# nikizadehgfdl/ocean_model_grid_generator

Measured on AMD Instinct MI355X. Metric: supergrid cells/sec (coords+metrics), 1/8° tripolar at 1/2/4/8 MI355X, higher is better.
Workload: dtype f64

## Files before the change

include/ogg_hip.h:

```cpp
#ifndef OGG_HIP_H
#define OGG_HIP_H

#ifdef __cplusplus
extern "C" {
#endif

#define OGG_OK 0
#define OGG_EORDER 1
#define OGG_ESHAPE 2
#define OGG_EHIP 3
#define OGG_ENOMEM 4
#define OGG_EARG 5

#define OGG_DP_ARC_LITERAL 0
#define OGG_DP_ARC_CHORD 1

#define OGG_SYM_DEFAULT 0
#define OGG_SYM_MIRROR 1
#define OGG_SYM_NONE 2

const char* ogg_last_error(void);
const char* ogg_version(void);
long ogg_abi_sizeof(int which);
int ogg_device_count(int* count);
// ... 177 lines not shown
    long workspace_bytes;
    int symmetry;
} ogg_dpole_band;
long ogg_dpole_band_workspace_bytes(int order, long Ni, long n_pt_rows);
int ogg_symmetry_coverage(int which, int order, long n, double lon0, double lon_dp, int symmetry, int* cell_writes, int* col_writes,
                          long* evaluated);
int ogg_supergrid_pass_dev(int n_latlon, const ogg_latlon_band* latlon, long ni1, double lon0, double lenlon, double Re, int metrics,
                           const ogg_bipolar_band* cap, const ogg_dpole_band* south_cap, void** events5, double* alg_bytes4,
                           void* stream);
int ogg_supergrid_pass_plan_dev(int n_latlon, const ogg_latlon_band* latlon, long ni1, double lon0, double lenlon, double Re, int metrics,
                                const ogg_bipolar_band* cap, const ogg_dpole_band* south_cap, void** plan_out);
int ogg_supergrid_pass_run_dev(void* plan, void** events5, double* alg_bytes4, void* stream);
int ogg_supergrid_pass_plan_destroy(void* plan);
long ogg_supergrid_pass_plan_slots(const void* plan);
long ogg_supergrid_pass_plan_carried_runs(const void* plan);
int ogg_supergrid_pass_plan_flags_dev(const void* plan, int* flags, void* stream);

int ogg_fill_dev(long n, double value, double* out, void* stream);
int ogg_bswap64_dev(long n, const void* src, void* dst, void* stream);
int ogg_libm_check_dev(int which, long n, const double* x, const double* y, unsigned long long* n_diff, void* stream);
#define OGG_MATH_DIV_PI180 0
#define OGG_MATH_RCP_C3 1
#define OGG_MATH_RSQRT_C3 2
#define OGG_MATH_ATAN_SERIES14 3
#define OGG_MATH_ATAN_SERIES17 4
#define OGG_MATH_ATAN_CAP 5
#define OGG_MATH_ATAN2_ANGLE 6
#define OGG_MATH_WAVE_PREV 7
#define OGG_MATH_WAVE_NEXT 8
#define OGG_MATH_WAVE_PREV_TAIL 9
// ... 372 lines not shown
```

ocean_model_grid_generator_amd/_lib.py:

```python
import ctypes
import os

import numpy as np

_HERE = os.path.dirname(os.path.abspath(__file__))
LIB_PATH = os.environ.get("OGG_LIB_PATH") or os.path.join(_HERE, "csrc", "libogg_hip.so")

OGG_OK, OGG_EORDER, OGG_ESHAPE, OGG_EHIP, OGG_ENOMEM, OGG_EARG = 0, 1, 2, 3, 4, 5
DP_ARC_LITERAL, DP_ARC_CHORD = 0, 1
SYM_DEFAULT, SYM_MIRROR, SYM_NONE = 0, 1, 2

MATH = {"div_pi180": 0, "rcp_c3": 1, "rsqrt_c3": 2, "atan_series14": 3, "atan_series17": 4, "atan_cap": 5, "atan2_angle": 6,
        "wave_prev": 7, "wave_next": 8, "wave_prev_tail": 9, "wave_next_tail": 10, "xcd_contiguous": 11, "lib_atan": 12, "atan_lib": 13, "wave_next_int": 14,
        "sin_tiny": 32, "asin_tiny": 33, "cos_cap": 34, "hom_arc": 35, "hom_tan": 36, "lib_sin": 37, "lib_asin": 38, "lib_cos": 39}

c_long, c_int, c_double, c_void_p, c_longlong = ctypes.c_long, ctypes.c_int, ctypes.c_double, ctypes.c_void_p, ctypes.c_longlong
_dp = ctypes.POINTER(ctypes.c_double)
_llp = ctypes.POINTER(ctypes.c_longlong)

class LatlonBand(ctypes.Structure):
    _fields_ = [("axis_kind", c_int), ("a0", c_double), ("len", c_double), ("denom", c_double), ("y0", c_longlong),
                ("lat1d", c_void_p), ("k0", c_long), ("n_pt_rows", c_long), ("n_cell_rows", c_long), ("x", c_void_p),
                ("y", c_void_p), ("dx", c_void_p), ("dy", c_void_p), ("area", c_void_p), ("angle", c_void_p)]

# ... 364 lines not shown
    "ogg_event_create": [ctypes.POINTER(c_void_p)],
    "ogg_event_destroy": [c_void_p],
    "ogg_event_record": [c_void_p, c_void_p],
    "ogg_event_elapsed_ms": [c_void_p, c_void_p, ctypes.POINTER(ctypes.c_float)],
    "ogg_stream_synchronize": [c_void_p],
}
STRING_GETTERS = ("ogg_last_error", "ogg_version")
LONG_GETTERS = {"ogg_abi_sizeof": [c_int],
                "ogg_bipolar_quad_workspace_bytes": [c_int, c_long, c_long],
                "ogg_displaced_pole_quad_workspace_bytes": [c_int, c_long, c_long],
                "ogg_displaced_pole_grid_workspace_bytes": [c_long, c_long],
                "ogg_dpole_band_workspace_bytes": [c_int, c_long, c_long],
                "ogg_latlon_rows_workspace_bytes": [c_int, ctypes.POINTER(LatlonBand), c_long],
                "ogg_supergrid_pass_plan_slots": [c_void_p],
                "ogg_supergrid_pass_plan_carried_runs": [c_void_p],
                "ogg_grid_quality_result_bytes": [],
                "ogg_grid_quality_workspace_bytes": [c_long, c_long],
                "ogg_topog_record_bytes": [],
                "ogg_topog_plane_record_bytes": [],
                "ogg_topog_band_out_rows": [ctypes.POINTER(TopogBand)],
                "ogg_topog_workspace_bytes": [],
                "ogg_xgrid_struct_bytes": [c_int],
                "ogg_xgrid_band_first_row": [ctypes.POINTER(XgridBand)],
                "ogg_xgrid_band_out_rows": [ctypes.POINTER(XgridBand)],
                "ogg_xgrid_band_next_rows": [ctypes.POINTER(XgridBand)],
                "ogg_xgrid_workspace_bytes": [ctypes.POINTER(XgridBand), ctypes.POINTER(XgridAtm)],
                "ogg_mask_struct_bytes": [c_int],
                "ogg_mask_workspace_bytes": [ctypes.POINTER(MaskParams)],
                "ogg_remap_struct_bytes": [c_int],
                "ogg_remap_workspace_bytes": [ctypes.POINTER(RemapParams)],
# ... 91 lines not shown
```

ocean_model_grid_generator_amd/csrc/ogg_latlon_fused_dev.h:

```cpp
#pragma once
#include <cmath>
#include <cstdlib>

#include "../../include/ogg_hip.h"
#include "ogg_common.h"
#include "ogg_math.h"

namespace {
using namespace ogg;

constexpr int LF_TX = 256;
constexpr int LF_ROWS = 32;
constexpr int LF_MAX_BANDS = 4;

struct RowScalars {
    double lat, sl, cl, dy;
};

struct FusedParams {
    int n_bands;
    ogg_latlon_band band[LF_MAX_BANDS];
    long strip0[LF_MAX_BANDS + 1];
    long ni1;
    double lon0, lenlon, Ni;
    int rows_per_block;
    double Re, Re2;
    int metrics;
    const RowScalars* row_tab;
    long row0[LF_MAX_BANDS + 1];
};

OGG_DEV double axis_lat(const ogg_latlon_band& b, long k, double Ni) {
    if (b.axis_kind == 0) return b.a0 + ((double)k * b.len) / b.denom;
    if (b.axis_kind == 1) {
        const double R = Ni / (2 * kPi);
        return atan(sinh((double)(b.y0 + k) / R)) * k180Pi;
    }
    return b.lat1d[k];
}

OGG_DEV RowScalars latlon_row_scalars(const FusedParams& f, const ogg_latlon_band& b, long j) {
    const long n_cell_rows = f.metrics ? b.n_cell_rows : 0;
    RowScalars r = {0.0, 0.0, 0.0, 0.0};
    if (j < b.n_pt_rows || j - 1 < n_cell_rows) {
        r.lat = axis_lat(b, b.k0 + j, f.Ni);
        const double lv = (0.5 * (r.lat + r.lat)) * kPi180;
        sincos(lv, &r.sl, &r.cl);
        if (j < n_cell_rows) {
            const double dyj = (axis_lat(b, b.k0 + j + 1, f.Ni) - r.lat) * kPi180;
            r.dy = f.Re * sqrt(dyj * dyj + 0.0);
        }
    }
    return r;
}

OGG_DEV void latlon_row_table_body(const FusedParams& f, long b, long n_wg) {
    const long n_rows = f.row0[f.n_bands];
    RowScalars* tab = const_cast<RowScalars*>(f.row_tab);
    for (long k = b * LF_TX + threadIdx.x; k < n_rows; k += n_wg * LF_TX) {
        int bi = 0;
        while (bi + 1 < f.n_bands && k >= f.row0[bi + 1]) ++bi;
        tab[k] = latlon_row_scalars(f, f.band[bi], k - f.row0[bi]);
    }
}
inline long latlon_row_table_blocks(const FusedParams& f) { return f.n_bands ? (f.row0[f.n_bands] + LF_TX - 1) / LF_TX : 0; }

struct ColScalars {
    double lon_c, dlam, hdlam, xdiff;
};

OGG_DEV ColScalars column_scalars(const FusedParams& p, long i) {
    const long ni1 = p.ni1, ni = ni1 - 1;
    const long ic = (i < ni1) ? i : ni;
    ColScalars c;
    c.lon_c = p.lon0 + ((double)ic * p.lenlon) / p.Ni;
    const double lon_r = p.lon0 + ((double)((ic + 1 < ni1) ? ic + 1 : ic) * p.lenlon) / p.Ni;
    const double lon_l = p.lon0 + ((double)((ic > 0) ? ic - 1 : 0) * p.lenlon) / p.Ni;
    c.dlam = mdist(lon_r, c.lon_c) * kPi180;
    c.hdlam = 0.5 * (c.dlam + c.dlam);
    if (i == 0)
        c.xdiff = lon_r - c.lon_c;
    else if (i == ni)
        c.xdiff = c.lon_c - lon_l;
    else
        c.xdiff = lon_r - lon_l;
    return c;
}

typedef double dbl2 __attribute__((ext_vector_type(2), aligned(8)));

template <bool FULL, bool NT>
OGG_DEV void store2(double* q, double a, double b, bool first, bool second) {
    if (FULL) {
        dbl2 v;
        v.x = a, v.y = b;
        if (NT)
            __builtin_nontemporal_store(v, reinterpret_cast<dbl2*>(q));
        else
            *reinterpret_cast<dbl2*>(q) = v;
    } else {
        if (NT) {
            if (first) __builtin_nontemporal_store(a, q);
            if (second) __builtin_nontemporal_store(b, q + 1);
        } else {
            if (first) q[0] = a;
            if (second) q[1] = b;
        }
    }
}

OGG_DEV double latlon_angle(double pa) {
    const double r = (__double2hiint(pa) < 0) ? kPi / kPi180 : 0.0 / kPi180;
    return (pa != pa) ? pa : r;
}

template <bool FULL, bool NT>
OGG_DEV void latlon_rows(const FusedParams& p, const ogg_latlon_band& b, const RowScalars* s_row, long js, int nrows, long n_cell_rows,
                         long i0, const ColScalars& c0, const ColScalars& c1) {
    const long ni1 = p.ni1, ni = ni1 - 1;
    const bool pt1 = i0 + 1 < ni1, ce0 = i0 < ni;
    double* __restrict__ px = b.x + (js * ni1 + i0);
    double* __restrict__ py = b.y + (js * ni1 + i0);
    double* __restrict__ pa = b.angle + (js * ni1 + i0);
    double* __restrict__ pdx = b.dx + (js * ni + i0);
    double* __restrict__ pdy = b.dy + (js * ni1 + i0);
    double* __restrict__ par = b.area + (js * ni + i0);
    for (int r = 0; r < nrows; ++r) {
        const long j = js + r;
        const RowScalars rs = s_row[r];
        store2<FULL, NT>(px, c0.lon_c, c1.lon_c, true, pt1);
        store2<FULL, NT>(py, rs.lat, rs.lat, true, pt1);
        store2<FULL, NT>(pa, latlon_angle(c0.xdiff * rs.cl), latlon_angle(c1.xdiff * rs.cl), true, pt1);
        if (p.metrics) {
            store2<FULL, NT>(pdx, p.Re * fabs(c0.dlam * rs.cl), p.Re * fabs(c1.dlam * rs.cl), ce0, false);
            if (j < n_cell_rows) {
                store2<FULL, NT>(pdy, rs.dy, rs.dy, true, pt1);
                const double ds = s_row[r + 1].sl - rs.sl;
                store2<FULL, NT>(par, p.Re2 * (c0.hdlam * ds), p.Re2 * (c1.hdlam * ds), ce0, false);
            }
        }
        px += ni1, py += ni1, pa += ni1, pdy += ni1;
// ... 7 lines not shown
    asm volatile("global_atomic_add %0, %1, %2, off sc0" : "=v"(ret) : "v"(counter), "v"(one) : "memory");
    return ret;
}
template <int LATER>
OGG_DEV unsigned ticket_answer(unsigned pending) {
    unsigned out;
    asm volatile("s_waitcnt vmcnt(%2)\n\tv_mov_b32 %0, %1" : "=v"(out) : "v"(pending), "n"(LATER) : "memory");
    return out;
}

constexpr int LF_COLS = 2 * LF_TX;
inline long latlon_gx(long ni1) { return (ni1 + LF_COLS - 1) / LF_COLS; }

template <bool NT, bool TAB = false>
OGG_DEV void latlon_fused_body(const FusedParams& p, RowScalars* s_row, long b, long gx, long gy, long strip_lo, long strip_hi,
                               unsigned* claims = nullptr, bool helper = false, int* s_claim = nullptr, bool pool = false) {
    const long v = xcd_contiguous(b, gx * gy);
    const long bx = v % gx, by = v / gx;
    const int tid = threadIdx.x;
    const long i0 = (bx * LF_TX + tid) * 2;
    const long ni1 = p.ni1, ni = ni1 - 1;
    const ColScalars c0 = column_scalars(p, i0), c1 = column_scalars(p, i0 + 1);
    const bool full = i0 + 1 < ni;
    const long per = (strip_hi - strip_lo + gy - 1) / gy;
    const long s_first = strip_lo + by * per, s_last = (s_first + per < strip_hi) ? s_first + per : strip_hi;
    unsigned* cnt = claims ? (pool ? claims + bx : claims + 2 * (by * gx + bx)) : nullptr;
    const unsigned n_pool = (unsigned)(strip_hi - strip_lo);
    if (pool) {
        if (tid == 0) {
            const unsigned t = atomicAdd(cnt, 1u);
            *s_claim = t < n_pool ? (int)t : -1;
        }
        __syncthreads();
    }
    long walked = 0;
    for (long strip = s_first;; ++strip) {
        unsigned asked;
        if (pool) {
            const int pick = *s_claim;
            if (pick < 0) break;
            strip = strip_lo + pick;
            if (tid == 0) asked = ticket_ask(cnt);
        } else if (cnt) {
            if (tid == 0) {
                const unsigned n = (unsigned)(s_last > s_first ? s_last - s_first : 0);
                int pick = -1;
                if (atomicAdd(cnt, 1u) < n) pick = helper ? (int)(n - 1u - atomicAdd(cnt + 1, 1u)) : (int)walked;
                *s_claim = pick;
            }
            __syncthreads();
            const int pick = *s_claim;
            if (pick < 0) break;
            strip = s_first + pick;
            ++walked;
        } else if (strip >= s_last) {
            break;
// ... 17 lines not shown
                    const double lv = (0.5 * (r.lat + r.lat)) * kPi180;
                    sincos(lv, &r.sl, &r.cl);
                }
                s_row[tid] = r;
            }
            __syncthreads();
            if (p.metrics && tid < nrows) {
                const long j = js + tid;
                if (j < n_cell_rows) {
                    const double dyj = (s_row[tid + 1].lat - s_row[tid].lat) * kPi180;
                    s_row[tid].dy = p.Re * sqrt(dyj * dyj + 0.0);
                }
            }
        }
        __syncthreads();
        if (full)
            latlon_rows<true, NT>(p, b, s_row, js, nrows, n_cell_rows, i0, c0, c1);
        else if (i0 < ni1)
            latlon_rows<false, NT>(p, b, s_row, js, nrows, n_cell_rows, i0, c0, c1);
        if (pool && tid == 0) {
            const unsigned t = nrows >= 6 ? ticket_answer<16>(asked) : nrows == 5 ? ticket_answer<12>(asked) : nrows == 4 ? ticket_answer<8>(asked)
                               : nrows == 3 ? ticket_answer<6>(asked) : ticket_answer<0>(asked);
            *s_claim = t < n_pool ? (int)t : -1;
        }
        __syncthreads();
    }
}

__global__ __launch_bounds__(LF_TX) void latlon_fused_kernel(FusedParams p) {
    __shared__ RowScalars s_row[LF_ROWS + 1];
    latlon_fused_body<false>(p, s_row, (long)blockIdx.y * gridDim.x + blockIdx.x, gridDim.x, gridDim.y, 0, p.strip0[p.n_bands]);
}

inline void set_rows_per_strip(FusedParams& p, long rpb) {
    rpb = rpb < 1 ? 1 : (rpb > LF_ROWS ? LF_ROWS : rpb);
    p.rows_per_block = (int)rpb;
    p.strip0[0] = 0;
// ... 37 lines not shown
```

ocean_model_grid_generator_amd/csrc/ogg_pass.hip:

```cpp
#include <cstring>
#include <new>
#include <vector>

#include "ogg_bipolar_dev.h"
#include "ogg_dpole_dev.h"
#include "ogg_latlon_fused_dev.h"

extern "C" long ogg_dpole_band_workspace_bytes(int order, long Ni, long n_pt_rows);

namespace {

constexpr int PASS_TX = 256;
static_assert(PASS_TX == LF_TX && PASS_TX == 64 * MESH_WAVES && PASS_TX == 64 * QS_WAVES && PASS_TX == 64 * DM_WAVES &&
                  PASS_TX == 64 * DQ_WAVES,
              "one workgroup shape for all roles");

struct LatlonShare {
    long n_wg;
    long gx, gy;
    long strip_lo, strip_hi;
    int nt;
    unsigned* claims;
    long n_help;
    int pool;
    long points;
};

union PassLds {
    RowScalars ll[LF_ROWS + 1];
    BpRow mesh[MESH_ROWS_MAX];
    DpMeshLds dmesh;
    QuadOutLds quad;
};

struct PassAParams {
    FusedParams ll;
    LatlonShare share;
    MeshParams mesh;
    long mesh_gx, n_mesh;
    QuadParams q;
    long n_tab;
    DpQuadParams dq;
    long n_dq_tab;
    int dq_order;
    DpMeshParams dm;
    long n_dm_reset;
    long n_ll_tab;
};

template <int N>
OGG_DEV void pass_table_roles(const PassAParams& a, long b) {
    if (b < a.n_tab) {
        bipolar_tables_body<N>(a.q, b);
        return;
    }
    b -= a.n_tab;
    if (b < a.n_dq_tab) {
        if (a.dq_order == 2)
            dpole_quad_tables_body<2>(a.dq, b, a.n_dq_tab);
        else
            dpole_quad_tables_body<4>(a.dq, b, a.n_dq_tab);
        return;
    }
    b -= a.n_dq_tab;
    if (b < a.n_dm_reset) {
        dpole_mesh_reset_body(a.dm, b, a.n_dm_reset);
        return;
    }
    b -= a.n_dm_reset;
    if (b < a.n_ll_tab) latlon_row_table_body(a.ll, b, a.n_ll_tab);
}

template <int N>
__global__ __launch_bounds__(PASS_TX) void pass_a_kernel(PassAParams a) {
    __shared__ PassLds lds;
    long b = blockIdx.x;
    if (b < a.share.n_wg) {
        if (a.share.nt)
            latlon_fused_body<true>(a.ll, lds.ll, b, a.share.gx, a.share.gy, a.share.strip_lo, a.share.strip_hi);
        else
            latlon_fused_body<false>(a.ll, lds.ll, b, a.share.gx, a.share.gy, a.share.strip_lo, a.share.strip_hi);
        return;
    }
    b -= a.share.n_wg;
    if (b < a.n_tab) {
        bipolar_tables_body<N>(a.q, b);
        return;
    }
    b -= a.n_tab;
    if (b < a.n_dq_tab) {
        if (a.dq_order == 2)
            dpole_quad_tables_body<2>(a.dq, b, a.n_dq_tab);
        else
            dpole_quad_tables_body<4>(a.dq, b, a.n_dq_tab);
        return;
    }
    b -= a.n_dq_tab;
    if (b < a.n_dm_reset) {
        dpole_mesh_reset_body(a.dm, b, a.n_dm_reset);
        return;
    }
    b -= a.n_dm_reset;
    if (b < a.n_ll_tab) {
        latlon_row_table_body(a.ll, b, a.n_ll_tab);
        return;
    }
    b -= a.n_ll_tab;
    if (b < a.n_mesh) bipolar_mesh_body<false>(a.mesh, lds.mesh, b % a.mesh_gx, b / a.mesh_gx);
}

struct PassBParams {
    FusedParams ll;
    LatlonShare share;
    MeshParams mesh;
    long mesh_gx, n_mesh;
    QuadParams q;
    QuadRange guard, fast;
    long n_guard, n_fast;
    DpMeshParams dm;
// ... 36 lines not shown
        for (int k = 0; k < 8; ++k) big[k] = ~0ull;
        if (hipMemcpyToSymbol(g_tl_first, big, 64) != hipSuccess) return 1;
        for (int k = 1; k < 5; ++k)
            if (hipMemcpyToSymbol(sym[k], z, 64) != hipSuccess) return 1;
    }
    return 0;
}
extern "C" int ogg_timeline_strips(unsigned long long* out512) {
    return hipMemcpyFromSymbol(out512, g_tl_strip_end, sizeof g_tl_strip_end) == hipSuccess ? 0 : 1;
}
#define OGG_TL_DONE(r) tl.done(r)
#else
#define OGG_TL_DONE(r)
#endif

template <int N, bool TAB>
__global__ __launch_bounds__(PASS_TX, TAB ? 4 : 1) void pass_b_kernel(PassBParams a) {
    __shared__ PassLds lds;
    __shared__ unsigned s_slot;
    __shared__ int s_claim;
#ifdef OGG_TIMELINE
    const Timeline tl;
#endif
    long b = blockIdx.x;
    if (b >= (long)gridDim.x - a.n_next) {
        pass_table_roles<N>(*a.next, b - ((long)gridDim.x - a.n_next));
        OGG_TL_DONE(7);
        return;
    }
    const long first_help = (long)gridDim.x - a.n_next - a.share.n_help;
    const bool helper = b >= first_help;
    if (b < a.share.n_wg || helper) {
        if (helper) {
            const long k = b - first_help, n = a.share.n_wg;
            long r = (k / 8) * 8 + (b % 8);
            b = r % n;
        }
        if (a.share.nt)
            latlon_fused_body<true, TAB>(a.ll, lds.ll, b, a.share.gx, a.share.gy, a.share.strip_lo, a.share.strip_hi, a.share.claims, helper, &s_claim, a.share.pool != 0);
        else
            latlon_fused_body<false, TAB>(a.ll, lds.ll, b, a.share.gx, a.share.gy, a.share.strip_lo, a.share.strip_hi, a.share.claims, helper, &s_claim, a.share.pool != 0);
        OGG_TL_DONE(helper ? 1 : 0);
        return;
    }
    b -= a.share.n_wg;
    int role = -1;
#pragma unroll
    for (int k = 0; k < N_ROLES; ++k) {
        const int r = a.order[k];
        const long n = (r == ROLE_BP_MESH) ? a.n_mesh : (r == ROLE_DP_MESH) ? a.n_dmesh : (r == ROLE_BP_GUARD) ? a.n_guard : (r == ROLE_BP_FAST) ? a.n_fast : a.n_dquad;
        if (role < 0) {
            if (b < n)
                role = r;
            else
                b -= n;
        }
// ... 40 lines not shown
    s.nt = alone ? 0 : (int)env_long("OGG_PASS_LL_NT", 1);
    if (hi <= lo) return s;
    const long points = (hi - lo) * ll.rows_per_block * ni1;
    s.points = points;
    if (pool < 0) pool = (int)env_long("OGG_PASS_LL_POOL", (light || points >= 16000000) ? 1 : 0);
    s.pool = pool;
    long max_wg = alone ? 2048
                        : (points >= 16000000 ? env_long("OGG_PASS_LL_WG", pool ? (light ? (points >= 48000000 ? 72 : (table ? 108 : 96)) : (table ? 96 : 60)) : (light ? 156 : 90))
                                              : (points >= 8000000 ? env_long("OGG_PASS_LL_WG_MID", pool ? (table ? 108 : 96) : (light ? 150 : 90))
                                                                   : env_long("OGG_PASS_LL_WG_SMALL", points >= 4000000 ? (pool ? (table ? 108 : 96) : (light ? 180 : 120))
                                                                                                                        : ((pool && table) ? 108 : 120))));
    long gy = hi - lo;
    if (s.gx * gy > max_wg) gy = (max_wg + s.gx - 1) / s.gx;
    s.gy = gy < 1 ? 1 : gy;
    s.n_wg = s.gx * s.gy;
    return s;
}

double latlon_strip_bytes(const FusedParams& ll, long lo, long hi) {
    const long ni1 = ll.ni1, ni = ni1 - 1;
    double bytes = 0.0;
    for (int k = 0; k < ll.n_bands; ++k) {
        const long s0 = ll.strip0[k] > lo ? ll.strip0[k] : lo, s1 = ll.strip0[k + 1] < hi ? ll.strip0[k + 1] : hi;
        if (s1 <= s0) continue;
        const ogg_latlon_band& b = ll.band[k];
        const long r0 = (s0 - ll.strip0[k]) * ll.rows_per_block;
        long r1 = (s1 - ll.strip0[k]) * ll.rows_per_block;
        if (r1 > b.n_pt_rows) r1 = b.n_pt_rows;
        const long ncell = ll.metrics ? b.n_cell_rows : 0;
        const long c1 = r1 < ncell ? r1 : ncell, c0 = r0 < ncell ? r0 : ncell;
        bytes += 8.0 * ((double)(r1 - r0) * (3 * ni1 + (ll.metrics ? ni : 0)) + (double)(c1 - c0) * (ni1 + ni));
    }
// ... 2 lines not shown

double dpole_mesh_bytes(const ogg_dpole_band& d) { return 8.0 * 3.0 * (double)d.n_pt_rows * (double)(d.Ni + 1); }
double dpole_quad_bytes(const ogg_dpole_band& d) {
    return 8.0 * ((double)d.n_pt_rows * (double)d.Ni + (double)d.n_cell_rows * (2.0 * (double)d.Ni + 1.0));
}

struct PassPlan {
    int order;
    PassAParams A;
    PassBParams B;
    QuadPlan qp;
    DpQuadParams dq;
    int dq_order;
    bool have_quad, dq_literal, launch_b;
    unsigned na, nb, nd;
    unsigned b_lds_pad;
    double alg_bytes[4];
};

template <int N>
int build_pass_plan(const FusedParams& ll, long ni1, int metrics, const ogg_bipolar_band* cap, const ogg_dpole_band* scap, PassPlan& P) {
    P = PassPlan{};
    P.order = N;
    const long n_strips_ll = ll.n_bands ? ll.strip0[ll.n_bands] : 0;
    const bool have_cap = cap && cap->n_pt_rows > 0;
    const bool have_quad = have_cap && metrics;
    const bool have_dp = scap && scap->n_pt_rows > 0;
    const bool have_dquad = have_dp && metrics;
    const bool dq_literal = have_dquad && scap->arc_form == OGG_DP_ARC_LITERAL;
    PassAParams& A = P.A;
    PassBParams& B = P.B;
    QuadPlan& qp = P.qp;
    A.ll = ll, B.ll = ll;
    if (have_cap) {
        A.mesh = MeshParams{cap->Ni, cap->Nj, cap->lat0_bp, cap->lon_bp, cap->j0, cap->n_pt_rows, cap->x, cap->y, nullptr, nullptr, cap->angle, MESH_ROWS, {}};
        const dim3 mg = mesh_grid(A.mesh, ogg::cap_symmetry(cap->symmetry) ? 1 : 0);
        A.mesh_gx = mg.x, A.n_mesh = (long)mg.x * mg.y;
    }
// ... 38 lines not shown
        A.n_mesh = 0;
    }
    {
        const double ni = (double)(ni1 - 1);
        const double mesh_bytes = have_cap ? 8.0 * 3.0 * (double)cap->n_pt_rows * (double)ni1 : 0.0;
        const double bq_bytes = have_quad ? 8.0 * (double)cap->n_cell_rows * (3.0 * ni + 1.0) : 0.0;
        P.alg_bytes[0] = latlon_strip_bytes(ll, 0, s1) + (launch_b ? 0.0 : mesh_bytes) + ((have_quad && qp.has_top) ? 8.0 * ni : 0.0);
        P.alg_bytes[1] = launch_b ? latlon_strip_bytes(ll, s1, n_strips_ll) + bq_bytes + mesh_bytes + (have_dp ? dpole_mesh_bytes(*scap) : 0.0) +
                                        ((have_dquad && !dq_literal) ? dpole_quad_bytes(*scap) : 0.0)
                                  : 0.0;
        P.alg_bytes[2] = 0.0;
        P.alg_bytes[3] = dq_literal ? dpole_quad_bytes(*scap) : 0.0;
    }
    A.share = make_share(ll, 0, s1, ni1, !have_cap && !have_dp);
    if (!(launch_b && ll.row_tab && n_strips_ll > 0)) A.ll.row_tab = nullptr, B.ll.row_tab = nullptr;
    A.n_ll_tab = B.ll.row_tab ? latlon_row_table_blocks(ll) : 0;
    P.na = (unsigned)(A.share.n_wg + A.n_tab + A.n_dq_tab + A.n_dm_reset + A.n_ll_tab + A.n_mesh);
    if (launch_b) {
        static const int quad_first[N_ROLES] = {ROLE_BP_FAST, ROLE_BP_GUARD, ROLE_DP_QUAD, ROLE_BP_MESH, ROLE_DP_MESH};
        static const int mesh_first[N_ROLES] = {ROLE_BP_MESH, ROLE_DP_MESH, ROLE_BP_GUARD, ROLE_BP_FAST, ROLE_DP_QUAD};
        const double quad_cells = (have_quad ? (double)cap->n_cell_rows * (double)cap->Ni : 0.0) +
                                  ((have_dquad && !dq_literal) ? (double)scap->n_cell_rows * (double)scap->Ni : 0.0);
        const int* dflt = quad_cells >= 2.0e6 ? quad_first : mesh_first;
        const char* ord = getenv("OGG_PASS_ORDER");
        for (int k = 0; k < N_ROLES; ++k)
            B.order[k] = (ord && strlen(ord) == N_ROLES && ord[k] >= '0' && ord[k] < '0' + N_ROLES) ? ord[k] - '0' : dflt[k];
        const bool light = have_cap && ogg::cap_symmetry(cap->symmetry) && B.n_dquad == 0;
        B.share = make_share(ll, s1, n_strips_ll, ni1, false, light, have_quad ? -1 : 0);
        if (B.share.pool && B.ll.row_tab && !getenv("OGG_LL_ROWS_PER_STRIP")) {
            const long rpb = env_long("OGG_PASS_LL_ROWS_TABLE", 6);
            if (rpb > 0 && rpb != B.ll.rows_per_block) {
                set_rows_per_strip(B.ll, rpb), set_rows_per_strip(A.ll, rpb);
                B.share = make_share(B.ll, 0, B.ll.strip0[B.ll.n_bands], ni1, false, light, have_quad ? -1 : 0, true);
            }
        }
        const long helpers = env_long("OGG_PASS_LL_HELPERS", (B.share.points >= 16000000 && !light) ? 2 : 0);
        if (B.share.pool && B.share.n_wg > 0 && B.share.gx <= QUAD_LL_CLAIM_WORDS) {
            B.share.claims = qp.p.ll_claims;
            B.share.n_help = B.share.n_wg * env_long("OGG_PASS_LL_POOL_HELPERS", (light || B.ll.row_tab) ? 0 : 1);
        } else if (B.share.pool) {
            B.share.pool = 0;
        } else if (have_quad && helpers > 0 && B.share.n_wg > 0 && 2 * B.share.n_wg <= QUAD_LL_CLAIM_WORDS) {
            B.share.claims = qp.p.ll_claims;
            B.share.n_help = B.share.n_wg * helpers;
        }
        P.nb = (unsigned)(B.share.n_wg + B.n_mesh + B.n_dmesh + B.n_guard + B.n_fast + B.n_dquad + B.share.n_help);
        P.b_lds_pad = (unsigned)env_long("OGG_PASS_B_LDS_PAD", (B.ll.row_tab && light && B.share.points >= 16000000) ? 41000 : 0);
    }
    P.nd = dq_literal ? (unsigned)(dq.gx * dq.n_chunks) : 0u;
    P.have_quad = have_quad, P.dq_literal = dq_literal, P.launch_b = launch_b;
    return OGG_OK;
}

template <int N>
int run_pass_plan(const PassPlan& P, hipEvent_t* ev, double* alg_bytes4, hipStream_t st, bool with_a = true, const PassAParams* next = nullptr,
                  long n_next = 0) {
    auto mark = [&](int k) -> int {
        if (ev && ev[k]) OGG_HIP_CHECK(hipEventRecord(ev[k], st));
        return OGG_OK;
    };
    if (alg_bytes4)
        for (int k = 0; k < 4; ++k) alg_bytes4[k] = P.alg_bytes[k];
    if (int e = mark(0)) return e;
    if (P.na > 0 && with_a) {
        pass_a_kernel<N><<<P.na, PASS_TX, 0, st>>>(P.A);
        OGG_LAUNCH_CHECK();
    }
    if (int e = mark(1)) return e;
    if (P.launch_b) {
        PassBParams b = P.B;
        if (next && n_next > 0) b.next = next, b.n_next = n_next;
        if (b.ll.row_tab)
            pass_b_kernel<N, true><<<P.nb + (unsigned)b.n_next, PASS_TX, P.b_lds_pad, st>>>(b);
        else
            pass_b_kernel<N, false><<<P.nb + (unsigned)b.n_next, PASS_TX, 0, st>>>(b);
        OGG_LAUNCH_CHECK();
    }
    if (int e = mark(2)) return e;
    if (P.have_quad) {
        if (int e = launch_quad_tail<N>(P.qp, st)) return e;
    }
    if (int e = mark(3)) return e;
    if (P.dq_literal) {
        if (P.dq_order == 2)
            pass_d_kernel<2><<<P.nd, PASS_TX, 0, st>>>(P.dq);
        else
            pass_d_kernel<4><<<P.nd, PASS_TX, 0, st>>>(P.dq);
        OGG_LAUNCH_CHECK();
    }
    return mark(4);
}

int build_pass_plan_any(int n_latlon, const ogg_latlon_band* latlon, long ni1, double lon0, double lenlon, double Re, int metrics,
                        const ogg_bipolar_band* cap, const ogg_dpole_band* south_cap, PassPlan& P, const RowScalars* row_tab = nullptr) {
    FusedParams ll;
    long points = 0;
    if (int e = plan_latlon(n_latlon, latlon, ni1, lon0, lenlon, Re, metrics, ll, points)) return e;
    ll.row_tab = row_tab;
    int order = 5;
    if (cap && cap->n_pt_rows > 0) {
        OGG_REQUIRE(cap->Ni + 1 == ni1, OGG_ESHAPE, "ogg_tripolar_pass: cap has %ld columns, the lat-lon bands %ld", cap->Ni + 1, ni1);
        OGG_REQUIRE(cap->Nj > 0 && cap->j0 >= 0 && cap->j0 + cap->n_pt_rows <= cap->Nj + 1, OGG_ESHAPE,
                    "ogg_tripolar_pass: cap rows %ld..%ld outside 0..%ld", cap->j0, cap->j0 + cap->n_pt_rows, cap->Nj);
        OGG_REQUIRE(cap->x && cap->y && cap->angle, OGG_EARG, "ogg_tripolar_pass: null cap output");
        if (metrics) {
            order = cap->order;
            OGG_REQUIRE(order >= 2 && order <= 5, OGG_EORDER, "Uncoded order");
            OGG_REQUIRE(cap->dx && (cap->n_cell_rows <= 0 || (cap->dy && cap->area)), OGG_EARG, "ogg_tripolar_pass: null cap metrics output");
            OGG_REQUIRE(cap->n_cell_rows >= 0 && cap->j0 + cap->n_cell_rows <= cap->Nj &&
                            (cap->n_pt_rows == cap->n_cell_rows ||
                             (cap->n_pt_rows == cap->n_cell_rows + 1 && cap->j0 + cap->n_cell_rows == cap->Nj)),
                        OGG_ESHAPE, "ogg_tripolar_pass: cap band j0=%ld cell rows=%ld point rows=%ld of Nj=%ld", cap->j0,
                        cap->n_cell_rows, cap->n_pt_rows, cap->Nj);
// ... 78 lines not shown
    P.A.q.dxq = P.qp.top_buf, P.A.q.top_out_row = 0;
    P.qp.p.top_src = P.qp.top_buf;
}

int build_pass_pipe(int n_latlon, const ogg_latlon_band* latlon, long ni1, double lon0, double lenlon, double Re, int metrics,
                    const ogg_bipolar_band* cap, const ogg_dpole_band* south_cap, PassPipe& H) {
    if (int e = build_pass_plan_any(n_latlon, latlon, ni1, lon0, lenlon, Re, metrics, cap, south_cap, H.slot[0])) return e;
    if (env_long("OGG_PASS_SLOTS", 2) < 2 || !H.slot[0].launch_b || H.slot[0].na == 0) return OGG_OK;
    OGG_HIP_CHECK(hipGetDevice(&H.device));
    const bool have_cap = cap && cap->n_pt_rows > 0 && cap->workspace, have_dp = south_cap && south_cap->n_pt_rows > 0;
    H.n_slots = 2;
    const long n_tab_rows = H.slot[0].A.ll.n_bands ? H.slot[0].A.ll.row0[H.slot[0].A.ll.n_bands] : 0;
    const bool row_table = n_tab_rows > 0 && env_long("OGG_PASS_LL_TABLE", 1) != 0;
    for (int k = 0; k < 2; ++k) {
        if (row_table) {
            OGG_HIP_CHECK(hipMalloc(&H.own_row_tab[k], (size_t)n_tab_rows * sizeof(RowScalars)));
            OGG_HIP_CHECK(hipMemset(H.own_row_tab[k], 0, (size_t)n_tab_rows * sizeof(RowScalars)));
        }
        ogg_bipolar_band c{};
        ogg_dpole_band d{};
        if (have_cap) {
            c = *cap;
            OGG_HIP_CHECK(hipMalloc(&H.own_ws[k][0], (size_t)cap->workspace_bytes));
            OGG_HIP_CHECK(hipMemset(H.own_ws[k][0], 0, (size_t)cap->workspace_bytes));
            c.workspace = H.own_ws[k][0];
        }
        if (have_dp) {
            d = *south_cap;
            OGG_HIP_CHECK(hipMalloc(&H.own_ws[k][1], (size_t)south_cap->workspace_bytes));
            OGG_HIP_CHECK(hipMemset(H.own_ws[k][1], 0, (size_t)south_cap->workspace_bytes));
            d.workspace = H.own_ws[k][1];
        }
// ... 139 lines not shown
    return OGG_OK;
}

extern "C" int ogg_supergrid_pass_run_dev(void* plan, void** events5, double* alg_bytes4, void* stream) {
    OGG_REQUIRE(plan, OGG_EARG, "ogg_supergrid_pass_run: null plan");
    return run_pass_pipe(*static_cast<PassPipe*>(plan), events5, alg_bytes4, stream);
}

extern "C" int ogg_supergrid_pass_plan_destroy(void* plan) {
    delete static_cast<PassPipe*>(plan);
    return OGG_OK;
}

extern "C" long ogg_supergrid_pass_plan_slots(const void* plan) { return plan ? static_cast<const PassPipe*>(plan)->n_slots : 0; }
extern "C" long ogg_supergrid_pass_plan_carried_runs(const void* plan) { return plan ? (long)static_cast<const PassPipe*>(plan)->carried_runs : 0; }

extern "C" int ogg_supergrid_pass_plan_flags_dev(const void* plan, int* flags, void* stream) {
    OGG_REQUIRE(plan && flags, OGG_EARG, "ogg_supergrid_pass_plan_flags: null pointer");
    const PassPipe& H = *static_cast<const PassPipe*>(plan);
    OGG_HIP_CHECK(hipStreamSynchronize(ogg::as_stream(stream)));
    int f = 0;
    for (int k = 0; k < H.n_slots; ++k) {
        const PassPlan& P = H.slot[k];
        unsigned w = 0u;
        if (P.B.n_dmesh > 0 && P.B.dm.ticket) {
            OGG_HIP_CHECK(hipMemcpy(&w, P.B.dm.ticket + 1, sizeof(w), hipMemcpyDeviceToHost));
            if (w) f |= 2;
        }
        if (P.dq_order && P.dq.ticket) {
            OGG_HIP_CHECK(hipMemcpy(&w, P.dq.ticket + 1, sizeof(w), hipMemcpyDeviceToHost));
// ... 25 lines not shown
```

ocean_model_grid_generator_amd/supergrid.py:

```python
import ctypes
import math
import os

import numpy as np

from . import _lib as L
from . import ocean_grid_generator as ogg

FIELDS = ("x", "y", "dx", "dy", "area", "angle_dx")


def band(n_rows, rank, world):
    return (n_rows * rank) // world, (n_rows * (rank + 1)) // world


def band_weighted(cost, rank, world, top_capacity=1.0, capacities=None):
    c = np.concatenate(([0.0], np.cumsum(np.asarray(cost, dtype=np.float64))))
    total = c[-1]
    caps = [1.0] * (world - 1) + [float(top_capacity)] if capacities is None else [float(v) for v in capacities]
    if len(caps) != world or min(caps) <= 0.0:
        raise ValueError("band_weighted: %d capacities for %d ranks (all must be positive)" % (len(caps), world))
    before = np.concatenate(([0.0], np.cumsum(caps)))

    def edge(r):
# ... 531 lines not shown
            L.call("ogg_supergrid_pass_plan_dev", len(bands), arr, p.Ni + 1, p.lon0, p.lenlon, p.Re, 0 if p.skip_metrics else 1, capref, scapref,
                   ctypes.byref(handle))
            self._pass_args = (bands, arr, cap, scap, handle)
            self._pass_run = L.load().ogg_supergrid_pass_run_dev
        handle = self._pass_args[4]
        if self.pass_events is None:
            rc = self._pass_run(handle, None, None, st)
            if rc:
                L.check(rc)
            return
        evs = self._event_pool.pop() if self._event_pool else self._new_events()
        self.pass_bytes = (ctypes.c_double * 4)()
        L.call("ogg_supergrid_pass_run_dev", handle, evs, self.pass_bytes, st)
        self.pass_events.append(evs)

    def pass_plan_info(self):
        if self._pass_args is None:
            return 0, 0
        lib = L.load()
        return int(lib.ogg_supergrid_pass_plan_slots(self._pass_args[4])), int(lib.ogg_supergrid_pass_plan_carried_runs(self._pass_args[4]))

    def replan(self):
        if self._pass_args is not None:
            L.call("ogg_supergrid_pass_plan_destroy", self._pass_args[4])
            self._pass_args = None

    def close(self):
        self.replan()

    def __del__(self):
        try:
            self.replan()
        except Exception:
            pass

# ... 840 lines not shown
```

Measured before the change: 126.6 billion.

## Hand out lat-lon work row-major across a sized persistent pool with column table

Adds a row-major work handout mode (pool=2) where a fixed number of persistent workgroups claim (strip, column-tile) units from one shared counter, switching column tiles on the fly. Column scalars are precomputed into a table appended to the row table so tile switches need no recomputation. A field-major store ordering is added but off by default, along with plan introspection. The aim is better load balance and sequential write locality for large light-cap grids, at the cost of contention on a single atomic counter and extra table-building work.

After: 122.4 billion. 0.967x the previous value.

```diff
diff --git a/include/ogg_hip.h b/include/ogg_hip.h
--- a/include/ogg_hip.h
+++ b/include/ogg_hip.h
@@ -215,6 +215,7 @@
 int ogg_supergrid_pass_plan_destroy(void* plan);
 long ogg_supergrid_pass_plan_slots(const void* plan);
 long ogg_supergrid_pass_plan_carried_runs(const void* plan);
+long ogg_supergrid_pass_plan_latlon_info(const void* plan, int what);
 int ogg_supergrid_pass_plan_flags_dev(const void* plan, int* flags, void* stream);
 
 int ogg_fill_dev(long n, double value, double* out, void* stream);
diff --git a/ocean_model_grid_generator_amd/_lib.py b/ocean_model_grid_generator_amd/_lib.py
--- a/ocean_model_grid_generator_amd/_lib.py
+++ b/ocean_model_grid_generator_amd/_lib.py
@@ -402,6 +402,7 @@
                 "ogg_latlon_rows_workspace_bytes": [c_int, ctypes.POINTER(LatlonBand), c_long],
                 "ogg_supergrid_pass_plan_slots": [c_void_p],
                 "ogg_supergrid_pass_plan_carried_runs": [c_void_p],
+                "ogg_supergrid_pass_plan_latlon_info": [c_void_p, c_int],
                 "ogg_grid_quality_result_bytes": [],
                 "ogg_grid_quality_workspace_bytes": [c_long, c_long],
                 "ogg_topog_record_bytes": [],
diff --git a/ocean_model_grid_generator_amd/csrc/ogg_latlon_fused_dev.h b/ocean_model_grid_generator_amd/csrc/ogg_latlon_fused_dev.h
--- a/ocean_model_grid_generator_amd/csrc/ogg_latlon_fused_dev.h
+++ b/ocean_model_grid_generator_amd/csrc/ogg_latlon_fused_dev.h
@@ -16,6 +16,8 @@
 struct RowScalars {
     double lat, sl, cl, dy;
 };
+
+struct ColScalars;
 
 struct FusedParams {
     int n_bands;
@@ -28,7 +30,9 @@
     int metrics;
     const RowScalars* row_tab;
     long row0[LF_MAX_BANDS + 1];
+    const ColScalars* col_tab;
 };
+OGG_HD long latlon_tab_cols(long ni1) { return (ni1 + 2 * LF_TX - 1) / (2 * LF_TX) * (2 * LF_TX); }
 
 OGG_DEV double axis_lat(const ogg_latlon_band& b, long k, double Ni) {
     if (b.axis_kind == 0) return b.a0 + ((double)k * b.len) / b.denom;
@@ -53,17 +57,6 @@
     }
     return r;
 }
-
-OGG_DEV void latlon_row_table_body(const FusedParams& f, long b, long n_wg) {
-    const long n_rows = f.row0[f.n_bands];
-    RowScalars* tab = const_cast<RowScalars*>(f.row_tab);
-    for (long k = b * LF_TX + threadIdx.x; k < n_rows; k += n_wg * LF_TX) {
-        int bi = 0;
-        while (bi + 1 < f.n_bands && k >= f.row0[bi + 1]) ++bi;
-        tab[k] = latlon_row_scalars(f, f.band[bi], k - f.row0[bi]);
-    }
-}
-inline long latlon_row_table_blocks(const FusedParams& f) { return f.n_bands ? (f.row0[f.n_bands] + LF_TX - 1) / LF_TX : 0; }
 
 struct ColScalars {
     double lon_c, dlam, hdlam, xdiff;
@@ -87,6 +80,25 @@
     return c;
 }
 
+template <bool COLS>
+OGG_DEV void latlon_row_table_body(const FusedParams& f, long b, long n_wg) {
+    const long n_rows = f.row0[f.n_bands], n_cols = (COLS && f.col_tab) ? latlon_tab_cols(f.ni1) : 0;
+    RowScalars* tab = const_cast<RowScalars*>(f.row_tab);
+    ColScalars* ctab = const_cast<ColScalars*>(f.col_tab);
+    for (long k = b * LF_TX + threadIdx.x; k < n_rows + n_cols; k += n_wg * LF_TX) {
+        if (COLS && k >= n_rows) {
+            ctab[k - n_rows] = column_scalars(f, k - n_rows);
+            continue;
+        }
+        int bi = 0;
+        while (bi + 1 < f.n_bands && k >= f.row0[bi + 1]) ++bi;
+        tab[k] = latlon_row_scalars(f, f.band[bi], k - f.row0[bi]);
+    }
+}
+inline long latlon_row_table_blocks(const FusedParams& f) {
+    return f.n_bands ? (f.row0[f.n_bands] + (f.col_tab ? latlon_tab_cols(f.ni1) : 0) + LF_TX - 1) / LF_TX : 0;
+}
+
 typedef double dbl2 __attribute__((ext_vector_type(2), aligned(8)));
 
 template <bool FULL, bool NT>
@@ -114,7 +126,14 @@
     return (pa != pa) ? pa : r;
 }
 
-template <bool FULL, bool NT>
+constexpr int LL_STORES_PER_ROW = 3;
+template <int NROWS>
+struct TicketLater {
+    static constexpr int value = NROWS >= 6 ? 16 : NROWS == 5 ? 12 : NROWS == 4 ? 8 : NROWS == 3 ? 6 : 0;
+    static_assert(value <= NROWS * LL_STORES_PER_ROW, "the counted wait for the ticket needs that many stores behind ticket_ask");
+};
+
+template <bool FULL, bool NT, bool FM = false>
 OGG_DEV void latlon_rows(const FusedParams& p, const ogg_latlon_band& b, const RowScalars* s_row, long js, int nrows, long n_cell_rows,
                          long i0, const ColScalars& c0, const ColScalars& c1) {
     const long ni1 = p.ni1, ni = ni1 - 1;
@@ -125,6 +144,34 @@
     double* __restrict__ pdx = b.dx + (js * ni + i0);
     double* __restrict__ pdy = b.dy + (js * ni1 + i0);
     double* __restrict__ par = b.area + (js * ni + i0);
+    if (FM) {
+        for (int r = 0; r < nrows; ++r, px += ni1) store2<FULL, NT>(px, c0.lon_c, c1.lon_c, true, pt1);
+        for (int r = 0; r < nrows; ++r, py += ni1) {
+            const double lat = s_row[r].lat;
+            store2<FULL, NT>(py, lat, lat, true, pt1);
+        }
+        for (int r = 0; r < nrows; ++r, pa += ni1) {
+            const double cl = s_row[r].cl;
+            store2<FULL, NT>(pa, latlon_angle(c0.xdiff * cl), latlon_angle(c1.xdiff * cl), true, pt1);
+        }
+        if (p.metrics) {
+            for (int r = 0; r < nrows; ++r, pdx += ni) {
+                const double cl = s_row[r].cl;
+                store2<FULL, NT>(pdx, p.Re * fabs(c0.dlam * cl), p.Re * fabs(c1.dlam * cl), ce0, false);
+            }
+            const long left = n_cell_rows - js;
+            const int ncell = left < 0 ? 0 : (left < nrows ? (int)left : nrows);
+            for (int r = 0; r < ncell; ++r, pdy += ni1) {
+                const double dy = s_row[r].dy;
+                store2<FULL, NT>(pdy, dy, dy, true, pt1);
+            }
+            for (int r = 0; r < ncell; ++r, par += ni) {
+                const double ds = s_row[r + 1].sl - s_row[r].sl;
+                store2<FULL, NT>(par, p.Re2 * (c0.hdlam * ds), p.Re2 * (c1.hdlam * ds), ce0, false);
+            }
+        }
+        return;
+    }
     for (int r = 0; r < nrows; ++r) {
         const long j = js + r;
         const RowScalars rs = s_row[r];
@@ -162,18 +209,20 @@
 
 template <bool NT, bool TAB = false>
 OGG_DEV void latlon_fused_body(const FusedParams& p, RowScalars* s_row, long b, long gx, long gy, long strip_lo, long strip_hi,
-                               unsigned* claims = nullptr, bool helper = false, int* s_claim = nullptr, bool pool = false) {
-    const long v = xcd_contiguous(b, gx * gy);
-    const long bx = v % gx, by = v / gx;
+                               unsigned* claims = nullptr, bool helper = false, int* s_claim = nullptr, int pool = 0, bool fm = false) {
+    const bool row_major = pool == 2;
+    const long v = row_major ? b : xcd_contiguous(b, gx * gy);
+    long bx = v % gx;
+    const long by = v / gx;
     const int tid = threadIdx.x;
-    const long i0 = (bx * LF_TX + tid) * 2;
+    long i0 = (bx * LF_TX + tid) * 2;
     const long ni1 = p.ni1, ni = ni1 - 1;
-    const ColScalars c0 = column_scalars(p, i0), c1 = column_scalars(p, i0 + 1);
-    const bool full = i0 + 1 < ni;
+    ColScalars c0 = column_scalars(p, i0), c1 = column_scalars(p, i0 + 1);
+    bool full = i0 + 1 < ni;
     const long per = (strip_hi - strip_lo + gy - 1) / gy;
     const long s_first = strip_lo + by * per, s_last = (s_first + per < strip_hi) ? s_first + per : strip_hi;
-    unsigned* cnt = claims ? (pool ? claims + bx : claims + 2 * (by * gx + bx)) : nullptr;
-    const unsigned n_pool = (unsigned)(strip_hi - strip_lo);
+    unsigned* cnt = claims ? (row_major ? claims : pool ? claims + bx : claims + 2 * (by * gx + bx)) : nullptr;
+    const unsigned n_pool = (unsigned)((strip_hi - strip_lo) * (row_major ? gx : 1));
     if (pool) {
         if (tid == 0) {
             const unsigned t = atomicAdd(cnt, 1u);
@@ -187,7 +236,22 @@
         if (pool) {
             const int pick = *s_claim;
             if (pick < 0) break;
-            strip = strip_lo + pick;
+            if (row_major) {
+                const unsigned u = (unsigned)__builtin_amdgcn_readfirstlane(pick), g = (unsigned)gx;
+                const long tile = u % g;
+                strip = strip_lo + u / g;
+                if (tile != bx) {
+                    bx = tile;
+                    i0 = (bx * LF_TX + tid) * 2;
+                    if (p.col_tab)
+                        c0 = p.col_tab[i0], c1 = p.col_tab[i0 + 1];
+                    else
+                        c0 = column_scalars(p, i0), c1 = column_scalars(p, i0 + 1);
+                    full = i0 + 1 < ni;
+                }
+            } else {
+                strip = strip_lo + pick;
+            }
             if (tid == 0) asked = ticket_ask(cnt);
         } else if (cnt) {
             if (tid == 0) {
@@ -235,13 +299,21 @@
             }
         }
         __syncthreads();
-        if (full)
+        if (fm) {
+            if (full)
+                latlon_rows<true, NT, true>(p, b, s_row, js, nrows, n_cell_rows, i0, c0, c1);
+            else if (i0 < ni1)
+                latlon_rows<false, NT, true>(p, b, s_row, js, nrows, n_cell_rows, i0, c0, c1);
+        } else if (full)
             latlon_rows<true, NT>(p, b, s_row, js, nrows, n_cell_rows, i0, c0, c1);
         else if (i0 < ni1)
             latlon_rows<false, NT>(p, b, s_row, js, nrows, n_cell_rows, i0, c0, c1);
         if (pool && tid == 0) {
-            const unsigned t = nrows >= 6 ? ticket_answer<16>(asked) : nrows == 5 ? ticket_answer<12>(asked) : nrows == 4 ? ticket_answer<8>(asked)
-                               : nrows == 3 ? ticket_answer<6>(asked) : ticket_answer<0>(asked);
+            const unsigned t = nrows >= 6    ? ticket_answer<TicketLater<6>::value>(asked)
+                               : nrows == 5 ? ticket_answer<TicketLater<5>::value>(asked)
+                               : nrows == 4 ? ticket_answer<TicketLater<4>::value>(asked)
+                               : nrows == 3 ? ticket_answer<TicketLater<3>::value>(asked)
+                                            : ticket_answer<TicketLater<0>::value>(asked);
             *s_claim = t < n_pool ? (int)t : -1;
         }
         __syncthreads();
diff --git a/ocean_model_grid_generator_amd/csrc/ogg_pass.hip b/ocean_model_grid_generator_amd/csrc/ogg_pass.hip
--- a/ocean_model_grid_generator_amd/csrc/ogg_pass.hip
+++ b/ocean_model_grid_generator_amd/csrc/ogg_pass.hip
@@ -23,7 +23,9 @@
     unsigned* claims;
     long n_help;
     int pool;
+    int field_major;
     long points;
+    long max_wg;
 };
 
 union PassLds {
@@ -48,7 +50,7 @@
     long n_ll_tab;
 };
 
-template <int N>
+template <int N, bool COLS>
 OGG_DEV void pass_table_roles(const PassAParams& a, long b) {
     if (b < a.n_tab) {
         bipolar_tables_body<N>(a.q, b);
@@ -68,10 +70,10 @@
         return;
     }
     b -= a.n_dm_reset;
-    if (b < a.n_ll_tab) latlon_row_table_body(a.ll, b, a.n_ll_tab);
-}
-
-template <int N>
+    if (b < a.n_ll_tab) latlon_row_table_body<COLS>(a.ll, b, a.n_ll_tab);
+}
+
+template <int N, bool COLS = false>
 __global__ __launch_bounds__(PASS_TX) void pass_a_kernel(PassAParams a) {
     __shared__ PassLds lds;
     long b = blockIdx.x;
@@ -102,7 +104,7 @@
     }
     b -= a.n_dm_reset;
     if (b < a.n_ll_tab) {
-        latlon_row_table_body(a.ll, b, a.n_ll_tab);
+        latlon_row_table_body<COLS>(a.ll, b, a.n_ll_tab);
         return;
     }
     b -= a.n_ll_tab;
@@ -169,7 +171,7 @@
 #define OGG_TL_DONE(r)
 #endif
 
-template <int N, bool TAB>
+template <int N, bool TAB, bool HO = false>
 __global__ __launch_bounds__(PASS_TX, TAB ? 4 : 1) void pass_b_kernel(PassBParams a) {
     __shared__ PassLds lds;
     __shared__ unsigned s_slot;
@@ -179,7 +181,7 @@
 #endif
     long b = blockIdx.x;
     if (b >= (long)gridDim.x - a.n_next) {
-        pass_table_roles<N>(*a.next, b - ((long)gridDim.x - a.n_next));
+        pass_table_roles<N, HO>(*a.next, b - ((long)gridDim.x - a.n_next));
         OGG_TL_DONE(7);
         return;
     }
@@ -191,10 +193,12 @@
             long r = (k / 8) * 8 + (b % 8);
             b = r % n;
         }
+        const int pool = HO ? a.share.pool : (a.share.pool != 0 ? 1 : 0);
+        const bool fm = HO && a.share.field_major != 0;
         if (a.share.nt)
-            latlon_fused_body<true, TAB>(a.ll, lds.ll, b, a.share.gx, a.share.gy, a.share.strip_lo, a.share.strip_hi, a.share.claims, helper, &s_claim, a.share.pool != 0);
+            latlon_fused_body<true, TAB>(a.ll, lds.ll, b, a.share.gx, a.share.gy, a.share.strip_lo, a.share.strip_hi, a.share.claims, helper, &s_claim, pool, fm);
         else
-            latlon_fused_body<false, TAB>(a.ll, lds.ll, b, a.share.gx, a.share.gy, a.share.strip_lo, a.share.strip_hi, a.share.claims, helper, &s_claim, a.share.pool != 0);
+            latlon_fused_body<false, TAB>(a.ll, lds.ll, b, a.share.gx, a.share.gy, a.share.strip_lo, a.share.strip_hi, a.share.claims, helper, &s_claim, pool, fm);
         OGG_TL_DONE(helper ? 1 : 0);
         return;
     }
@@ -265,8 +269,12 @@
     if (s.gx * gy > max_wg) gy = (max_wg + s.gx - 1) / s.gx;
     s.gy = gy < 1 ? 1 : gy;
     s.n_wg = s.gx * s.gy;
+    s.max_wg = max_wg;
     return s;
 }
+
+bool handout_row_default(long points, bool light, bool table) { return light && table && points >= 16000000; }
+long field_major_default() { return 0; }
 
 double latlon_strip_bytes(const FusedParams& ll, long lo, long hi) {
     const long ni1 = ll.ni1, ni = ni1 - 1;
@@ -299,6 +307,7 @@
     int dq_order;
     bool have_quad, dq_literal, launch_b;
     unsigned na, nb, nd;
+    int planned_rows;
     unsigned b_lds_pad;
     double alg_bytes[4];
 };
@@ -307,6 +316,7 @@
 int build_pass_plan(const FusedParams& ll, long ni1, int metrics, const ogg_bipolar_band* cap, const ogg_dpole_band* scap, PassPlan& P) {
     P = PassPlan{};
     P.order = N;
+    P.planned_rows = ll.rows_per_block;
     const long n_strips_ll = ll.n_bands ? ll.strip0[ll.n_bands] : 0;
     const bool have_cap = cap && cap->n_pt_rows > 0;
     const bool have_quad = have_cap && metrics;
@@ -375,8 +385,7 @@
     }
     A.share = make_share(ll, 0, s1, ni1, !have_cap && !have_dp);
     if (!(launch_b && ll.row_tab && n_strips_ll > 0)) A.ll.row_tab = nullptr, B.ll.row_tab = nullptr;
-    A.n_ll_tab = B.ll.row_tab ? latlon_row_table_blocks(ll) : 0;
-    P.na = (unsigned)(A.share.n_wg + A.n_tab + A.n_dq_tab + A.n_dm_reset + A.n_ll_tab + A.n_mesh);
+    A.ll.col_tab = nullptr, B.ll.col_tab = nullptr;
     if (launch_b) {
         static const int quad_first[N_ROLES] = {ROLE_BP_FAST, ROLE_BP_GUARD, ROLE_DP_QUAD, ROLE_BP_MESH, ROLE_DP_MESH};
         static const int mesh_first[N_ROLES] = {ROLE_BP_MESH, ROLE_DP_MESH, ROLE_BP_GUARD, ROLE_BP_FAST, ROLE_DP_QUAD};
@@ -388,26 +397,41 @@
             B.order[k] = (ord && strlen(ord) == N_ROLES && ord[k] >= '0' && ord[k] < '0' + N_ROLES) ? ord[k] - '0' : dflt[k];
         const bool light = have_cap && ogg::cap_symmetry(cap->symmetry) && B.n_dquad == 0;
         B.share = make_share(ll, s1, n_strips_ll, ni1, false, light, have_quad ? -1 : 0);
+        long claim_words = env_long("OGG_PASS_LL_CLAIM_WORDS", QUAD_LL_CLAIM_WORDS);
+        claim_words = claim_words < 0 ? 0 : (claim_words > QUAD_LL_CLAIM_WORDS ? QUAD_LL_CLAIM_WORDS : claim_words);
+        if (B.share.pool && !(have_quad && B.share.n_wg > 0 && B.share.gx <= claim_words))
+            B.share = make_share(ll, s1, n_strips_ll, ni1, false, light, 0);
         if (B.share.pool && B.ll.row_tab && !getenv("OGG_LL_ROWS_PER_STRIP")) {
             const long rpb = env_long("OGG_PASS_LL_ROWS_TABLE", 6);
             if (rpb > 0 && rpb != B.ll.rows_per_block) {
                 set_rows_per_strip(B.ll, rpb), set_rows_per_strip(A.ll, rpb);
-                B.share = make_share(B.ll, 0, B.ll.strip0[B.ll.n_bands], ni1, false, light, have_quad ? -1 : 0, true);
+                B.share = make_share(B.ll, 0, B.ll.strip0[B.ll.n_bands], ni1, false, light, 1, true);
             }
         }
         const long helpers = env_long("OGG_PASS_LL_HELPERS", (B.share.points >= 16000000 && !light) ? 2 : 0);
-        if (B.share.pool && B.share.n_wg > 0 && B.share.gx <= QUAD_LL_CLAIM_WORDS) {
+        if (B.share.pool) {
             B.share.claims = qp.p.ll_claims;
+            const char* ho = getenv("OGG_PASS_LL_HANDOUT");
+            const bool row_dflt = handout_row_default(B.share.points, light, B.ll.row_tab != nullptr);
+            const bool row_major = ho ? strcmp(ho, "row") == 0 : row_dflt;
+            const long n_units = (B.share.strip_hi - B.share.strip_lo) * B.share.gx;
+            if (row_major && n_units < 0x7fffffffL) {
+                B.share.pool = 2;
+                const long wg = row_dflt ? env_long("OGG_PASS_LL_WG", B.share.points >= 48000000 ? 161 : 120) : B.share.max_wg;
+                B.share.n_wg = wg < 1 ? 1 : (wg < n_units ? wg : n_units);
+            }
+            B.share.field_major = (int)env_long("OGG_PASS_LL_FIELD_MAJOR", field_major_default()) != 0;
             B.share.n_help = B.share.n_wg * env_long("OGG_PASS_LL_POOL_HELPERS", (light || B.ll.row_tab) ? 0 : 1);
-        } else if (B.share.pool) {
-            B.share.pool = 0;
-        } else if (have_quad && helpers > 0 && B.share.n_wg > 0 && 2 * B.share.n_wg <= QUAD_LL_CLAIM_WORDS) {
+        } else if (have_quad && helpers > 0 && B.share.n_wg > 0 && 2 * B.share.n_wg <= claim_words) {
             B.share.claims = qp.p.ll_claims;
             B.share.n_help = B.share.n_wg * helpers;
         }
+        if (B.share.pool == 2 && B.ll.row_tab) A.ll.col_tab = B.ll.col_tab = ll.col_tab;
         P.nb = (unsigned)(B.share.n_wg + B.n_mesh + B.n_dmesh + B.n_guard + B.n_fast + B.n_dquad + B.share.n_help);
         P.b_lds_pad = (unsigned)env_long("OGG_PASS_B_LDS_PAD", (B.ll.row_tab && light && B.share.points >= 16000000) ? 41000 : 0);
     }
+    A.n_ll_tab = B.ll.row_tab ? latlon_row_table_blocks(A.ll) : 0;
+    P.na = (unsigned)(A.share.n_wg + A.n_tab + A.n_dq_tab + A.n_dm_reset + A.n_ll_tab + A.n_mesh);
     P.nd = dq_literal ? (unsigned)(dq.gx * dq.n_chunks) : 0u;
     P.have_quad = have_quad, P.dq_literal = dq_literal, P.launch_b = launch_b;
     return OGG_OK;
@@ -424,17 +448,25 @@
         for (int k = 0; k < 4; ++k) alg_bytes4[k] = P.alg_bytes[k];
     if (int e = mark(0)) return e;
     if (P.na > 0 && with_a) {
-        pass_a_kernel<N><<<P.na, PASS_TX, 0, st>>>(P.A);
+        if (P.A.ll.col_tab)
+            pass_a_kernel<N, true><<<P.na, PASS_TX, 0, st>>>(P.A);
+        else
+            pass_a_kernel<N, false><<<P.na, PASS_TX, 0, st>>>(P.A);
         OGG_LAUNCH_CHECK();
     }
     if (int e = mark(1)) return e;
     if (P.launch_b) {
         PassBParams b = P.B;
         if (next && n_next > 0) b.next = next, b.n_next = n_next;
-        if (b.ll.row_tab)
-            pass_b_kernel<N, true><<<P.nb + (unsigned)b.n_next, PASS_TX, P.b_lds_pad, st>>>(b);
+        const bool ho = b.share.pool == 2 || b.share.field_major;
+        if (b.ll.row_tab && ho)
+            pass_b_kernel<N, true, true><<<P.nb + (unsigned)b.n_next, PASS_TX, P.b_lds_pad, st>>>(b);
+        else if (b.ll.row_tab)
+            pass_b_kernel<N, true, false><<<P.nb + (unsigned)b.n_next, PASS_TX, P.b_lds_pad, st>>>(b);
+        else if (ho)
+            pass_b_kernel<N, false, true><<<P.nb + (unsigned)b.n_next, PASS_TX, 0, st>>>(b);
         else
-            pass_b_kernel<N, false><<<P.nb + (unsigned)b.n_next, PASS_TX, 0, st>>>(b);
+            pass_b_kernel<N, false, false><<<P.nb + (unsigned)b.n_next, PASS_TX, 0, st>>>(b);
         OGG_LAUNCH_CHECK();
     }
     if (int e = mark(2)) return e;
@@ -458,6 +490,7 @@
     long points = 0;
     if (int e = plan_latlon(n_latlon, latlon, ni1, lon0, lenlon, Re, metrics, ll, points)) return e;
     ll.row_tab = row_tab;
+    ll.col_tab = (row_tab && ll.n_bands) ? reinterpret_cast<const ColScalars*>(row_tab + ll.row0[ll.n_bands]) : nullptr;
     int order = 5;
     if (cap && cap->n_pt_rows > 0) {
         OGG_REQUIRE(cap->Ni + 1 == ni1, OGG_ESHAPE, "ogg_tripolar_pass: cap has %ld columns, the lat-lon bands %ld", cap->Ni + 1, ni1);
@@ -566,8 +599,9 @@
     const bool row_table = n_tab_rows > 0 && env_long("OGG_PASS_LL_TABLE", 1) != 0;
     for (int k = 0; k < 2; ++k) {
         if (row_table) {
-            OGG_HIP_CHECK(hipMalloc(&H.own_row_tab[k], (size_t)n_tab_rows * sizeof(RowScalars)));
-            OGG_HIP_CHECK(hipMemset(H.own_row_tab[k], 0, (size_t)n_tab_rows * sizeof(RowScalars)));
+            const size_t tab_bytes = (size_t)n_tab_rows * sizeof(RowScalars) + (size_t)latlon_tab_cols(ni1) * sizeof(ColScalars);
+            OGG_HIP_CHECK(hipMalloc(&H.own_row_tab[k], tab_bytes));
+            OGG_HIP_CHECK(hipMemset(H.own_row_tab[k], 0, tab_bytes));
         }
         ogg_bipolar_band c{};
         ogg_dpole_band d{};
@@ -737,6 +771,22 @@
 
 extern "C" long ogg_supergrid_pass_plan_slots(const void* plan) { return plan ? static_cast<const PassPipe*>(plan)->n_slots : 0; }
 extern "C" long ogg_supergrid_pass_plan_carried_runs(const void* plan) { return plan ? (long)static_cast<const PassPipe*>(plan)->carried_runs : 0; }
+extern "C" long ogg_supergrid_pass_plan_latlon_info(const void* plan, int what) {
+    if (!plan) return -1;
+    const PassPlan& P = static_cast<const PassPipe*>(plan)->slot[0];
+    const LatlonShare& s = P.launch_b ? P.B.share : P.A.share;
+    switch (what) {
+        case 0: return (P.launch_b ? P.B.ll : P.A.ll).rows_per_block;
+        case 1: return P.planned_rows;
+        case 2: return s.n_wg;
+        case 3: return s.claims ? s.pool : 0;
+        case 4: return s.field_major;
+        case 5: return s.gx;
+        case 6: return s.n_help;
+        case 7: return s.nt;
+        default: return -1;
+    }
+}
 
 extern "C" int ogg_supergrid_pass_plan_flags_dev(const void* plan, int* flags, void* stream) {
     OGG_REQUIRE(plan && flags, OGG_EARG, "ogg_supergrid_pass_plan_flags: null pointer");
diff --git a/ocean_model_grid_generator_amd/supergrid.py b/ocean_model_grid_generator_amd/supergrid.py
--- a/ocean_model_grid_generator_amd/supergrid.py
+++ b/ocean_model_grid_generator_amd/supergrid.py
@@ -569,11 +569,17 @@
         L.call("ogg_supergrid_pass_run_dev", handle, evs, self.pass_bytes, st)
         self.pass_events.append(evs)
 
-    def pass_plan_info(self):
+    def pass_plan_info(self, detail=False):
         if self._pass_args is None:
-            return 0, 0
+            return {} if detail else (0, 0)
         lib = L.load()
-        return int(lib.ogg_supergrid_pass_plan_slots(self._pass_args[4])), int(lib.ogg_supergrid_pass_plan_carried_runs(self._pass_args[4]))
+        h = self._pass_args[4]
+        slots, carried = int(lib.ogg_supergrid_pass_plan_slots(h)), int(lib.ogg_supergrid_pass_plan_carried_runs(h))
+        if not detail:
+            return slots, carried
+        v = [int(lib.ogg_supergrid_pass_plan_latlon_info(h, k)) for k in range(8)]
+        return {"slots": slots, "carried_runs": carried, "rows_per_strip": v[0], "planned_rows_per_strip": v[1], "ll_wg": v[2],
+                "handout": ("owned", "tile", "row")[v[3]], "field_major": bool(v[4]), "column_tiles": v[5], "helpers": v[6], "nt": bool(v[7])}
 
     def replan(self):
         if self._pass_args is not None:
```
